# lyndonchan/wsss-analysis

Measured on AMD Instinct MI355X. Metric: images/sec CAM+CRF pseudo-labels, VOC2012 321x321, higher is better.
Workload: dtype f16x3; 1 GPU; resnet50 CAM + dense-CRF (M=21, 10 mean-field iters), 321x321, batch 32 images (=64 samples) per GPU, image-sharded; batch_images=32, num_classes=20, parallelism=image-sharded x1, no collective, steps_per_rank=239

## Files before the change

### include/wsscam.h

```cpp
#ifndef WSSCAM_H
#define WSSCAM_H

#include <stddef.h>
#include <stdint.h>

#ifdef __cplusplus
extern "C" {
#endif

#define WSC_VERSION 100

typedef enum wsc_status {
    WSC_OK = 0,
    WSC_ERR_INVALID = -1,
    WSC_ERR_NO_DEVICE = -2,
    WSC_ERR_HIP = -3,
    WSC_ERR_MISSING_KEY = -4,
    WSC_ERR_SHAPE = -5,
    WSC_ERR_NOMEM = -6,
    WSC_ERR_KEY_RANGE = -7,
    WSC_ERR_CAPACITY = -8,
    WSC_ERR_RANGE = -9
} wsc_status;

typedef enum wsc_arch {
    WSC_ARCH_RESNET50_CAM = 0,
    WSC_ARCH_VGG16_CAM = 1,
    WSC_ARCH_M7_CAM = 2,
    WSC_ARCH_RESNET50_IRN = 3,
    WSC_ARCH_VGG16_IRN = 4,
    WSC_ARCH_M7_IRN = 5,
    WSC_ARCH_DEEPLAB_LFOV = 6,
    WSC_ARCH_DEEPLAB_ASPP = 7
} wsc_arch;

typedef enum wsc_precision {
    WSC_PREC_BF16 = 0,
    WSC_PREC_BF16X3 = 1,
    WSC_PREC_F16 = 2,
    WSC_PREC_F16X3 = 3,
    WSC_PREC_F32 = 4
} wsc_precision;

typedef struct wsc_ctx wsc_ctx;
typedef struct wsc_net wsc_net;
typedef enum {
    WSC_OPT_CRF_GAUSS_ON_CHIP = 0,
    WSC_OPT_CRF_FUSED_BLUR = 1,
    WSC_OPT_CRF_BLUR_ON_CHIP = 2,
    WSC_OPT_CRF_RANK_BALLOT = 3,
    WSC_OPT_CRF_EMBED_FULL = 4,
    WSC_OPT_RW_TILED = 5,
    WSC_OPT_STEM_POOL_FUSED = 6,
    WSC_OPT_CONV_WINDOW = 7,
    WSC_OPT_CAM_HEAD_STREAM = 8,
    WSC_OPT_CRF_MSG_IN_UPDATE = 9,
    WSC_OPT_COUNT = 10
} wsc_option;

typedef struct wsc_crf wsc_crf;
typedef struct wsc_crf_v wsc_crf_v;

typedef struct wsc_tensor_desc {
    const char *name;
    const float *data;
    int32_t ndim;
    int64_t shape[4];
} wsc_tensor_desc;


int wsc_version(void);
const char *wsc_last_error(void);

int wsc_ctx_create(int device, void *stream, wsc_ctx **out);
void wsc_ctx_destroy(wsc_ctx *ctx);
int wsc_ctx_set_option(wsc_ctx *ctx, int option, int value);
int wsc_sync(wsc_ctx *ctx);
int wsc_ctx_range_status(wsc_ctx *ctx, int *flag_out, int clear);
int wsc_ctx_wait(wsc_ctx *ctx, wsc_ctx *other);
int wsc_ctx_mark(wsc_ctx *ctx, int slot);
int wsc_ctx_wait_mark(wsc_ctx *ctx, int slot);
int wsc_ctx_wait_for_mark(wsc_ctx *ctx, wsc_ctx *other, int slot);
int wsc_device_info(wsc_ctx *ctx, char *arch_name, size_t arch_name_len, int *num_cus);

int wsc_malloc(wsc_ctx *ctx, size_t bytes, void **dptr_out);
int wsc_free(wsc_ctx *ctx, void *dptr);
int wsc_memcpy_h2d(wsc_ctx *ctx, void *dst_dev, const void *src_host, size_t bytes);
int wsc_memcpy_d2h(wsc_ctx *ctx, void *dst_host, const void *src_dev, size_t bytes);
int wsc_memset(wsc_ctx *ctx, void *dst_dev, int value, size_t bytes);
int wsc_host_alloc(wsc_ctx *ctx, size_t bytes, void **host_out);
int wsc_host_free(wsc_ctx *ctx, void *host);
int wsc_host_write_segments(const char *path, int n, const void *const *ptrs, const size_t *sizes);
int wsc_memcpy_h2d_async(wsc_ctx *ctx, void *dst_dev, const void *src_pinned_host, size_t bytes);
int wsc_memcpy_d2h_async(wsc_ctx *ctx, void *dst_pinned_host, const void *src_dev, size_t bytes);

int wsc_timer_begin(wsc_ctx *ctx);
int wsc_timer_end(wsc_ctx *ctx, float *ms_out);

int wsc_profile_begin(wsc_ctx *ctx);
int wsc_profile_end(wsc_ctx *ctx, int max_classes, int32_t *calls_out, float *total_ms_out, double *work_out,
                    int *n_classes_out);
const char *wsc_profile_class_name(int cls);


int wsc_net_create(wsc_ctx *ctx, int arch, const wsc_tensor_desc *weights, int n_weights,
                   int num_classes, int precision, wsc_net **out);
void wsc_net_destroy(wsc_net *net);
int wsc_net_cam_size(const wsc_net *net, int S, int *h_out);
int wsc_net_feat_channels(const wsc_net *net, int *f_out);

int wsc_net_forward_cam(wsc_ctx *ctx, const wsc_net *net, const float *x_dev, int B, int S,
                        float *cam_dev, float *score_dev);
int wsc_net_cam_size_hw(const wsc_net *net, int H, int W, int *h_out, int *w_out);
int wsc_net_forward_cam_hw(wsc_ctx *ctx, const wsc_net *net, const float *x_dev, int B, int H, int W, float *cam_dev,
                           float *score_dev);

int wsc_net_forward_features(wsc_ctx *ctx, const wsc_net *net, const float *x_dev ,
                             int N, int S, float *feat_dev);

int wsc_net_forward_edge(wsc_ctx *ctx, const wsc_net *net, const float *x_dev, int B, int S, int feat_h, int feat_w,
                         float *edge_dev, float *dp_dev);
int wsc_net_edge_size(const wsc_net *net, int S, int *edge_hw, int *dp_hw);
int wsc_net_forward_edge_raw(wsc_ctx *ctx, const wsc_net *net, const float *x_dev, int N, int S, float *edge_dev, float *dp_dev);

int wsc_rw_propagate(wsc_ctx *ctx, const float *x_dev, const float *edge_dev, int K, int h, int w,
                     const int32_t *dirs_host, const int32_t *path_start_host, const int32_t *path_yx_host, int D,
                     float beta, int n_steps, float *rw_dev);
int wsc_rw_propagate_batch(wsc_ctx *ctx, int n_img, const int32_t *K_host, const int32_t *h_host,
                           const int32_t *w_host, const float *x_dev, const float *edge_dev,
                           const int32_t *dirs_host, const int32_t *path_start_host, const int32_t *path_yx_host,
                           int D, float beta, int n_steps, float *rw_dev);

int wsc_net_forward_gradcam(wsc_ctx *ctx, const wsc_net *net, const float *x_dev, int N, int S, int relu,
                            float *cams_dev, float *score_dev);

#define WSC_CONV_GENERIC 0x100
int wsc_conv2d_nchw(wsc_ctx *ctx, const float *x_dev, int N, int Cin, int H, int W, const float *w_host,
                    int Cout, int kh, int kw, int stride, int pad, const float *scale_host,
                    const float *shift_host, const float *residual_dev, int relu, int precision,
                    float *y_dev);
// ... 246 lines not shown
```

### wsss-analysis_amd/csrc/common.h

```cpp
#pragma once
#include <hip/hip_runtime.h>
#include <assert.h>
#include <stdint.h>
#include <map>
#include <string>
#include <unordered_map>
#include <vector>

#include "../../include/wsscam.h"

typedef uint16_t bf16_t;

typedef __bf16 bf16x8_t __attribute__((ext_vector_type(8)));
typedef _Float16 f16x8_t __attribute__((ext_vector_type(8)));
typedef float f32x16_t __attribute__((ext_vector_type(16)));
typedef float f32x4_t __attribute__((ext_vector_type(4)));

__host__ __device__ inline bf16_t f32_to_bf16(float f) {
    union { float f; uint32_t u; } v;
    v.f = f;
    uint32_t u = v.u;
    if ((u & 0x7fffffffu) > 0x7f800000u) return (bf16_t)((u >> 16) | 0x40);
    u += 0x7fffu + ((u >> 16) & 1u);
    return (bf16_t)(u >> 16);
// ... 33 lines not shown
__host__ __device__ inline float f16_to_f32(uint16_t h) {
#if defined(__HIP_DEVICE_COMPILE__)
    return (float)__builtin_bit_cast(_Float16, h);
#else
    union { float f; uint32_t u; } o, magic;
    magic.u = 113u << 23;
    const uint32_t shifted_exp = 0x7c00u << 13;
    o.u = ((uint32_t)h & 0x7fffu) << 13;
    const uint32_t exp = shifted_exp & o.u;
    o.u += (127u - 15u) << 23;
    if (exp == shifted_exp) o.u += (128u - 16u) << 23;
    else if (exp == 0) { o.u += 1u << 23; o.f -= magic.f; }
    o.u |= ((uint32_t)h & 0x8000u) << 16;
    return o.f;
#endif
}
__host__ __device__ inline uint16_t f32_to_h16(float f, int fmt) { return fmt ? f32_to_f16(f) : f32_to_bf16(f); }
__host__ __device__ inline float h16_to_f32(uint16_t h, int fmt) { return fmt ? f16_to_f32(h) : bf16_to_f32(h); }

void wsc_set_error(const char *fmt, ...);
#define WSC_HIP(expr)                                                                          \
    do {                                                                                       \
        hipError_t _e = (expr);                                                                \
        if (_e != hipSuccess) {                                                                \
            wsc_set_error("%s:%d: %s failed: %s", __FILE__, __LINE__, #expr,                   \
                          hipGetErrorString(_e));                                              \
            return WSC_ERR_HIP;                                                                \
        }                                                                                      \
    } while (0)
#define WSC_CHECK(cond, code, ...)                                                             \
    do {                                                                                       \
        if (!(cond)) {                                                                         \
            wsc_set_error(__VA_ARGS__);                                                        \
            return (code);                                                                     \
        }                                                                                      \
    } while (0)
#define WSC_TRY(expr)                                                                          \
    do {                                                                                       \
        int _s = (expr);                                                                       \
        if (_s != WSC_OK) return _s;                                                           \
    } while (0)

enum WscKernelClass {
    WSC_K_CONV256 = 0,
    WSC_K_CONV128,
    WSC_K_CONV64,
    WSC_K_CONV_SMALLCIN,
    WSC_K_POOL_MISC,
    WSC_K_CAM_TAIL,
    WSC_K_CRF_BUILD,
    WSC_K_GAUSS_MSG,
    WSC_K_BLUR,
    WSC_K_SLICE_UPDATE,
    WSC_K_CRF_MISC,
    WSC_K_WGRAD,
    WSC_K_GRAD_MISC,
    WSC_K_COUNT
};
struct WscProfRecord {
    int cls;
    double work;
    hipEvent_t e0, e1;
};

struct WscGaussCache;
void wsc_gauss_cache_destroy(WscGaussCache *cache);
struct wsc_ctx {
    int device = 0;
    hipStream_t stream = nullptr;
    bool own_stream = false;
    int num_cus = 0;
    std::string arch;
    void *ws = nullptr;
    size_t ws_bytes = 0;
    static constexpr int PIN_SLOTS = 8;
    struct PinSlot {
        void *p = nullptr;
        size_t bytes = 0;
        hipEvent_t ev = nullptr;
        bool busy = false;
    };
    PinSlot pin_ring[PIN_SLOTS];
    int pin_next = 0;
    int opt[WSC_OPT_COUNT] = {1, 1, 1, 0, 0, -1, 1, 1, 1, 1};
    void *zero_page = nullptr;
    unsigned *range_host = nullptr, *range_dev = nullptr;
    hipEvent_t ev0 = nullptr, ev1 = nullptr;
    hipEvent_t join_ev = nullptr;
    hipEvent_t marks[8] = {};
    bool mark_set[8] = {};
    hipStream_t aux_stream = nullptr;
    hipEvent_t fork_ev = nullptr, aux_done_ev = nullptr;
    bool profiling = false;
    std::vector<WscProfRecord> prof;
    std::vector<hipEvent_t> prof_pool;
    std::multimap<size_t, void *> free_blocks;
    std::unordered_map<void *, size_t> live_blocks;
    WscGaussCache *gauss_cache = nullptr;
};
int wsc_ctx_workspace(wsc_ctx *ctx, size_t bytes, void **out);
int wsc_ctx_range_check(wsc_ctx *ctx);
__device__ __forceinline__ unsigned half2_at_ceiling(unsigned hw) { return (hw & 0x7fff7fffu) + 0x04010401u; }
struct WscKernelTimer {
    wsc_ctx *ctx;
    int idx = -1;
    WscKernelTimer(wsc_ctx *c, int cls, double work);
    ~WscKernelTimer();
};
int wsc_ctx_cached_alloc(wsc_ctx *ctx, size_t bytes, void **out);
void wsc_ctx_cached_free(wsc_ctx *ctx, void *p);
struct WscCachedGuard {
    wsc_ctx *ctx;
    void *p;
    WscCachedGuard(wsc_ctx *c, void *q) : ctx(c), p(q) {}
    WscCachedGuard(const WscCachedGuard &) = delete;
    WscCachedGuard &operator=(const WscCachedGuard &) = delete;
    void free_now() {
        if (p) wsc_ctx_cached_free(ctx, p);
        p = nullptr;
    }
    ~WscCachedGuard() { free_now(); }
};
int wsc_ctx_upload_small(wsc_ctx *ctx, void *dst_dev, const void *src_host, size_t bytes);
class WscStagedTable {
  public:
    explicit WscStagedTable(wsc_ctx *c) : ctx(c) {}
    WscStagedTable(const WscStagedTable &) = delete;
    WscStagedTable &operator=(const WscStagedTable &) = delete;
    ~WscStagedTable() { release(); }
    size_t add(const void *src, size_t bytes);
    template <class T> size_t add(const std::vector<T> &v) { return add(v.data(), v.size() * sizeof(T)); }
    int upload();
    template <class T> T *at(size_t off) const { return reinterpret_cast<T *>(dev + off); }
    int read_back(size_t off, void *dst, size_t bytes);
    void release() { wsc_ctx_cached_free(ctx, dev); dev = nullptr; }
  private:
    wsc_ctx *ctx;
    std::vector<char> host;
    char *dev = nullptr;
};
template <int NV> __device__ __forceinline__ void block_sum(double (&v)[NV], double *scratch) {
#pragma unroll
    for (int k = 0; k < NV; ++k)
        for (int off = 32; off > 0; off >>= 1) v[k] += __shfl_xor(v[k], off, 64);
    const int wave = threadIdx.x >> 6, n_waves = blockDim.x >> 6;
    __syncthreads();
    if ((threadIdx.x & 63) == 0)
        for (int k = 0; k < NV; ++k) scratch[wave * NV + k] = v[k];
    __syncthreads();
#pragma unroll
    for (int k = 0; k < NV; ++k) {
        double s = 0.0;
        for (int w = 0; w < n_waves; ++w) s += scratch[w * NV + k];
        v[k] = s;
    }
}

int wsc_set_max_dynamic_lds(wsc_ctx *ctx, const void *fn, int bytes);

constexpr int CONV_FMT_F32 = 2;
inline int conv_fmt(wsc_precision prec) {
    if (prec == WSC_PREC_F32) return CONV_FMT_F32;
    return (prec == WSC_PREC_F16 || prec == WSC_PREC_F16X3) ? 1 : 0;
}
inline size_t conv_elem_bytes(wsc_precision prec) { return prec == WSC_PREC_F32 ? sizeof(float) : sizeof(bf16_t); }
inline int conv_split(wsc_precision prec) { return prec == WSC_PREC_BF16X3 ? 1 : (prec == WSC_PREC_F16X3 ? 2 : 0); }

// ... 262 lines not shown
```

### wsss-analysis_amd/csrc/crf.hip

```cpp
#include "common.h"

#include <atomic>
#include <cmath>
#include <cstring>
#include <memory>

namespace {

constexpr unsigned long long EMPTY_KEY = 0xFFFFFFFFFFFFFFFFull;
typedef float f32x2_t __attribute__((ext_vector_type(2)));

struct LatticeDev {
    int d = 0;
    int rep = 1;
    int rows = 0;
    int32_t *offset = nullptr;
    float *bary = nullptr;
    float *norm = nullptr;
    int2 *nbr = nullptr;
    int32_t *tslot_start = nullptr;
    int2 *slot_desc = nullptr;
    float *tent_w = nullptr;
    uint8_t *tent_p = nullptr;
    int32_t *row_slot_start = nullptr;
    int n_tiles = 0, n_slots = 0;
    bool sorted_dest = false;
    long long n_pix = 0;
    int M_cur = 0;
    float alpha = 0.f;
    int32_t *tile_rows = nullptr;
    int2 *tile_pstart = nullptr;
    int32_t *tile_list = nullptr;
    int n_tiles_occ = 0;
    int4 *gt_cnt = nullptr;
    int2 *gt_rows = nullptr;
    uint4 *gt_nbr = nullptr;
    uint4 *gt_pix = nullptr;
    int gt_stride = 0;
    std::vector<int32_t> v_per_image;
    int32_t *img_row = nullptr;
    int max_img_rows = 0;
    uint32_t *part_row = nullptr;
    bool bl_ok = false;
    int2 *bl_blk = nullptr;
    int bl_cap = 0;
    mutable std::vector<int2> bl_blk_host;
    mutable int bl_M = -1, bl_nblk = 0;
    mutable size_t bl_lds = 0;
};

constexpr int TILE_W = 16, TILE_H = 16, TILE_PIX = TILE_W * TILE_H;
static_assert(TILE_PIX <= 256, "an entry's pixel index is stored in one byte");
constexpr int SLOT_ENT = 32;
constexpr int SORT_MAX = 2048;
static_assert(TILE_PIX * 6 <= SORT_MAX && SORT_MAX <= 65535, "tile too large for the in-LDS grouping");

struct TileGeom {
    int H, W, ntx, nty, tpi;
};
__host__ __device__ inline TileGeom make_geom(int H, int W) {
    TileGeom g;
    g.H = H; g.W = W;
    g.ntx = (W + TILE_W - 1) / TILE_W;
    g.nty = (H + TILE_H - 1) / TILE_H;
    g.tpi = g.ntx * g.nty;
    return g;
}
struct TileBox {
    int x0, y0, cw, ch;
    int ebase;
};
__host__ __device__ inline TileBox tile_box(const TileGeom &g, int j) {
    const unsigned ty = (unsigned)j / (unsigned)g.ntx, tx = (unsigned)j - ty * (unsigned)g.ntx;
    TileBox b;
    b.x0 = (int)(tx * (unsigned)g.W / (unsigned)g.ntx);
    b.y0 = (int)(ty * (unsigned)g.H / (unsigned)g.nty);
    b.cw = (int)((tx + 1) * (unsigned)g.W / (unsigned)g.ntx) - b.x0;
    b.ch = (int)((ty + 1) * (unsigned)g.H / (unsigned)g.nty) - b.y0;
    b.ebase = b.y0 * g.W + b.x0 * b.ch;
    return b;
}
static_assert(TILE_W <= 26 && TILE_PIX <= 4096, "tile_div_magic range");
__host__ __device__ inline unsigned tile_div_magic(int cw) { return (65536u + (unsigned)cw - 1u) / (unsigned)cw; }

struct CtxBlocks {
    wsc_ctx *ctx;
    std::vector<void *> ptrs;
    explicit CtxBlocks(wsc_ctx *c) : ctx(c) {}
    CtxBlocks(CtxBlocks &&o) noexcept : ctx(o.ctx), ptrs(std::move(o.ptrs)) { o.ptrs.clear(); }
    ~CtxBlocks() { release(); }
    template <class T>
    int alloc(size_t bytes, T **out) {
        void *p = nullptr;
        WSC_TRY(wsc_ctx_cached_alloc(ctx, bytes, &p));
        ptrs.push_back(p);
        *out = static_cast<T *>(p);
        return WSC_OK;
    }
    void take(CtxBlocks &&o) {
        ptrs.insert(ptrs.end(), o.ptrs.begin(), o.ptrs.end());
        o.ptrs.clear();
    }
    void release() {
        for (void *p : ptrs) wsc_ctx_cached_free(ctx, p);
        ptrs.clear();
    }
};

struct GaussEntry {
    int H, W;
    float sxy;
    LatticeDev L;
    CtxBlocks blocks;
    int users = 0;
    unsigned long long last_use = 0;
    bool fuse_pending = true;
};
constexpr int GAUSS_CACHE_MAX = 64;
std::atomic<unsigned long long> g_gauss_use_clock{0};

}

struct wsc_crf {
    wsc_ctx *ctx = nullptr;
    int B = 0, H = 0, W = 0, N = 0;
    LatticeDev lat[2];
    uint4 *pix_rec = nullptr;
    uint32_t *pix_rec_b = nullptr;
    CtxBlocks blocks;
    GaussEntry *gauss = nullptr;
// ... 899 lines not shown
                        while (hi - lo > 1) {
                            const int mid = (lo + hi) >> 1;
                            if (rss_l[mid] <= pp) lo = mid;
                            else hi = mid;
                        }
                        single = rss_l[lo + 1] - rss_l[lo] == 1;
                    }
                    if (single) {
                        val[(unsigned)(r0 + lo) * (unsigned)LP + l] = v[u];
                    } else {
#pragma unroll
                        for (int k = 0; k < 4; ++k)
                            atomicAdd(&acc[lo * 32 + 4 * l + k], (unsigned long long)(long long)__float2int_rn(v[u][k] * PFIX_SCALE));
                    }
                }
            }
        }
    }
    __syncthreads();
    if (tr < gpb) {
        for (int row = tr; row < nr; row += gpb) {
            const int n = rss_l[row + 1] - rss_l[row];
            if (n == 1) continue;
            f32x4_t o = {0.f, 0.f, 0.f, 0.f};
            if (n > 1) {
#pragma unroll
                for (int k = 0; k < 4; ++k) o[k] = (float)(long long)acc[row * 32 + 4 * l + k] * PFIX_INV;
            }
            val[(unsigned)(r0 + row) * (unsigned)LP + l] = o;
        }
    }
}


__global__ __launch_bounds__(256) void blur1_kernel(const float *__restrict__ in, const int2 *__restrict__ nbr,
                                                    int rows, float *__restrict__ out) {
    for (int row = blockIdx.x * blockDim.x + threadIdx.x; row < rows; row += gridDim.x * blockDim.x) {
        const int2 nb = nbr[row];
        out[row] = row == 0 ? 0.f : in[row] + 0.5f * (in[nb.x] + in[nb.y]);
    }
}

__global__ __launch_bounds__(256) void blur4_kernel(const f32x4_t *__restrict__ in, const int2 *__restrict__ nbr,
                                                    int LP, int rows_local, int rep, f32x4_t *__restrict__ out) {
    const int rpb = 256 / LP;
    const int tr = threadIdx.x / LP;
    const int l = threadIdx.x - tr * LP;
    if (tr >= rpb) return;
    constexpr int U = 4;
    long long rbeg, rend;
    int rk;
    xcd_range_rep(rows_local, rep, rk, rbeg, rend);
    in += (size_t)rk * rows_local * LP;
    out += (size_t)rk * rows_local * LP;
    for (long long row0 = rbeg + tr; row0 < rend; row0 += U * rpb) {
        int2 nb[U];
        f32x4_t c[U], a[U], b[U];
#pragma unroll
        for (int u = 0; u < U; ++u) {
            const long long row = row0 + u * rpb;
            nb[u] = row < rend ? nbr[row] : make_int2(0, 0);
        }
#pragma unroll
        for (int u = 0; u < U; ++u) {
            const long long row = row0 + u * rpb;
            c[u] = in[(unsigned)(row < rend ? row : 0) * (unsigned)LP + l];
            a[u] = in[(unsigned)nb[u].x * (unsigned)LP + l];
            b[u] = in[(unsigned)nb[u].y * (unsigned)LP + l];
        }
#pragma unroll
        for (int u = 0; u < U; ++u) {
            const long long row = row0 + u * rpb;
            if (row < rend) {
                f32x4_t o;
#pragma unroll
                for (int k = 0; k < 4; ++k) o[k] = row == 0 ? 0.f : c[u][k] + 0.5f * (a[u][k] + b[u][k]);
                out[(unsigned)row * (unsigned)LP + l] = o;
            }
        }
    }
}

constexpr int BL_THREADS = 1024;
constexpr int BL_NVAR = 5;
constexpr int BL_VAR[BL_NVAR][2] = {{4, 4}, {4, 10}, {3, 13}, {2, 20}, {1, 26}};
inline int blur_lds_variant(int rows) {
    for (int v = 0; v < BL_NVAR; ++v)
        if (rows <= BL_VAR[v][1] * BL_THREADS && (size_t)(rows + 1) * BL_VAR[v][0] * 4 <= 160 * 1024 && rows < 65535) return v;
    return -1;
}
struct BlurLdsArgs {
    const int2 *nbr;
    const int32_t *img_row;
    const int2 *blk;
    float *val;
    int Mp, M, rows, npass;
};
template <int GW> struct FloatRun { float v[GW]; };
typedef float f32x3u_t __attribute__((ext_vector_type(3), aligned(4)));
template <int GW>
__device__ __forceinline__ FloatRun<GW> load_run(const float *q) {
    FloatRun<GW> r;
    if constexpr (GW == 4) {
        const f32x4_t x = *reinterpret_cast<const f32x4_t *>(q);
        r.v[0] = x[0]; r.v[1] = x[1]; r.v[2] = x[2]; r.v[3] = x[3];
    } else if constexpr (GW == 3) {
        const f32x3u_t x = *reinterpret_cast<const f32x3u_t *>(q);
        r.v[0] = x[0]; r.v[1] = x[1]; r.v[2] = x[2];
    } else if constexpr (GW == 2) {
        const f32x2_t x = *reinterpret_cast<const f32x2_t *>(q);
        r.v[0] = x[0]; r.v[1] = x[1];
    } else {
        r.v[0] = q[0];
    }
    return r;
}
template <int GW>
__device__ __forceinline__ void store_run(float *q, const FloatRun<GW> &r) {
    if constexpr (GW == 4) *reinterpret_cast<f32x4_t *>(q) = f32x4_t{r.v[0], r.v[1], r.v[2], r.v[3]};
    else if constexpr (GW == 3) {
        f32x3u_t x;
        x[0] = r.v[0]; x[1] = r.v[1]; x[2] = r.v[2];
        *reinterpret_cast<f32x3u_t *>(q) = x;
    } else if constexpr (GW == 2) *reinterpret_cast<f32x2_t *>(q) = f32x2_t{r.v[0], r.v[1]};
    else q[0] = r.v[0];
}
template <int GW, int RPT>
__device__ __forceinline__ void blur_lds_body(const BlurLdsArgs &p, float *pl, int img, int grp) {
    const int r0 = p.img_row[img], nr = p.img_row[img + 1] - r0;
    const int stride = nr + 1;
    const int c0 = grp * GW;
    const int tid = (int)threadIdx.x;
    float *vb = p.val + (size_t)r0 * p.Mp + c0;
    unsigned nb[RPT];
    auto load_idx = [&](int pass) {
        const int2 *q = p.nbr + (size_t)pass * p.rows + r0;
        constexpr int CH = RPT < 10 ? RPT : 10;
#pragma unroll
        for (int i0 = 0; i0 < RPT; i0 += CH) {
            int2 raw[CH];
#pragma unroll
            for (int i = 0; i < CH; ++i) {
                const int r = tid + (i0 + i) * BL_THREADS;
                raw[i] = (i0 + i < RPT && r < nr) ? q[r] : make_int2(0, 0);
            }
#pragma unroll
            for (int i = 0; i < CH; ++i)
                if (i0 + i < RPT)
                    nb[i0 + i] = (unsigned)(raw[i].x ? raw[i].x - r0 : nr) | ((unsigned)(raw[i].y ? raw[i].y - r0 : nr) << 16);
        }
    };
    load_idx(0);
#pragma unroll
    for (int i = 0; i < RPT; ++i) {
        const int r = tid + i * BL_THREADS;
        if (r < nr) {
            FloatRun<GW> run;
            if (GW == 3 && c0 + GW > p.Mp) {
#pragma unroll
                for (int g = 0; g < GW; ++g) run.v[g] = c0 + g < p.Mp ? vb[(size_t)r * p.Mp + g] : 0.f;
            } else {
                run = load_run<GW>(vb + (size_t)r * p.Mp);
            }
#pragma unroll
            for (int g = 0; g < GW; ++g) pl[g * stride + r] = c0 + g < p.M ? run.v[g] : 0.f;
        }
    }
    if (tid < GW) pl[tid * stride + nr] = 0.f;
    __syncthreads();
    float o[RPT][GW];
    for (int pass = 0; pass < p.npass; ++pass) {
#pragma unroll
        for (int i = 0; i < RPT; ++i) {
            const int r = tid + i * BL_THREADS;
            const int rc = r < nr ? r : nr;
            const int l1 = (int)(nb[i] & 0xffffu), l2 = (int)(nb[i] >> 16);
#pragma unroll
            for (int g = 0; g < GW; ++g) o[i][g] = pl[g * stride + rc] + 0.5f * (pl[g * stride + l1] + pl[g * stride + l2]);
        }
        if (pass + 1 < p.npass) load_idx(pass + 1);
        else break;
        __syncthreads();
#pragma unroll
        for (int i = 0; i < RPT; ++i) {
            const int r = tid + i * BL_THREADS;
            if (r < nr) {
#pragma unroll
                for (int g = 0; g < GW; ++g) pl[g * stride + r] = o[i][g];
            }
        }
        __syncthreads();
    }
#pragma unroll
    for (int i = 0; i < RPT; ++i) {
        const int r = tid + i * BL_THREADS;
        if (r < nr) {
            if (c0 + GW <= p.M) {
                FloatRun<GW> run;
#pragma unroll
                for (int g = 0; g < GW; ++g) run.v[g] = o[i][g];
                store_run<GW>(vb + (size_t)r * p.Mp, run);
            } else {
#pragma unroll
                for (int g = 0; g < GW; ++g)
                    if (c0 + g < p.M) vb[(size_t)r * p.Mp + g] = o[i][g];
            }
        }
    }
}
__global__ __launch_bounds__(BL_THREADS) void blur_lds_kernel(BlurLdsArgs p) {
    extern __shared__ float pl[];
    const int2 w = p.blk[blockIdx.x];
    if (w.x < 0) return;
    const int img = w.x & 0xffffff;
    switch (w.x >> 24) {
    case 0: blur_lds_body<BL_VAR[0][0], BL_VAR[0][1]>(p, pl, img, w.y); break;
    case 1: blur_lds_body<BL_VAR[1][0], BL_VAR[1][1]>(p, pl, img, w.y); break;
    case 2: blur_lds_body<BL_VAR[2][0], BL_VAR[2][1]>(p, pl, img, w.y); break;
    case 3: blur_lds_body<BL_VAR[3][0], BL_VAR[3][1]>(p, pl, img, w.y); break;
    default: blur_lds_body<BL_VAR[4][0], BL_VAR[4][1]>(p, pl, img, w.y); break;
    }
}

constexpr int GTI = 12, GTJ = 12, GBI = GTI + 4, GBJ = GTJ + 4;
constexpr int GLH = 6;

__global__ void gauss_ij_kernel(const unsigned long long *__restrict__ rowkey, int rows, int2 *__restrict__ ij,
                                int *__restrict__ bbox ) {
    for (int row = 1 + blockIdx.x * blockDim.x + threadIdx.x; row < rows; row += gridDim.x * blockDim.x) {
        int key[2];
        unpack_key<2>(rowkey[row], key);
        const int a = 2 * key[0] + key[1], b = key[0] + 2 * key[1];
        if (a % 3 != 0 || b % 3 != 0) atomicOr(&bbox[4], 1);
        const int i = a / 3, j = b / 3;
        ij[row] = make_int2(i, j);
        atomicMin(&bbox[0], i);
        atomicMin(&bbox[1], j);
        atomicMax(&bbox[2], i);
        atomicMax(&bbox[3], j);
    }
}

__global__ void gauss_tile_fill_kernel(const int2 *__restrict__ ij, int rows, int imin, int jmin, int nti, int ntj,
                                       int32_t *__restrict__ tile_rows, int32_t *__restrict__ occ) {
    for (int row = 1 + blockIdx.x * blockDim.x + threadIdx.x; row < rows; row += gridDim.x * blockDim.x) {
        const int i = ij[row].x - imin, j = ij[row].y - jmin;
        occ[(i / GTI) * ntj + j / GTJ] = 1;
        for (int ti = (i - GTI - 1 >= 0 ? (i - GTI - 1) / GTI : 0); ti <= (i + 2) / GTI && ti < nti; ++ti) {
            const int li = i - ti * GTI + 2;
            if (li < 0 || li >= GBI) continue;
            for (int tj = (j - GTJ - 1 >= 0 ? (j - GTJ - 1) / GTJ : 0); tj <= (j + 2) / GTJ && tj < ntj; ++tj) {
                const int lj = j - tj * GTJ + 2;
                if (lj < 0 || lj >= GBJ) continue;
                tile_rows[((long long)ti * ntj + tj) * (GBI * GBJ) + li * GBJ + lj] = row;
            }
        }
    }
}

__global__ void gauss_tile_pstart_kernel(const int32_t *__restrict__ tile_rows, const int32_t *__restrict__ row_slot_start,
                                         long long total, int2 *__restrict__ tile_pstart) {
    for (long long i = (long long)blockIdx.x * blockDim.x + threadIdx.x; i < total; i += (long long)gridDim.x * blockDim.x) {
        const int row = tile_rows[i];
        tile_pstart[i] = row ? make_int2(row_slot_start[row], row_slot_start[row + 1] - row_slot_start[row]) : make_int2(0, 0);
    }
}

__global__ __launch_bounds__(GBI * GBJ) void blur3_tile_kernel(const f32x4_t *__restrict__ in, const int32_t *__restrict__ tile_rows,
                                                         const int32_t *__restrict__ tile_list, int n_occ, int LP,
                                                         int rows_local, int rep, f32x4_t *__restrict__ out,
                                                         const f32x4_t *__restrict__ part, const int2 *__restrict__ tile_pstart,
                                                         int n_slots) {
    constexpr int P = GBI * GBJ;
    constexpr int PS = P + 1;
    __shared__ f32x4_t b0[GLH * PS];
    const int nb = gridDim.x, bid = blockIdx.x;
    const int xcd = bid & 7, qq = nb >> 3, rr = nb & 7;
    const int lb = (xcd < rr ? xcd * (qq + 1) : rr * (qq + 1) + (xcd - rr) * qq) + (bid >> 3);
    const int k = lb / n_occ, t = lb - k * n_occ;
    if (in) in += (size_t)k * rows_local * LP;
    if (part) part += (size_t)k * n_slots * LP;
    out += (size_t)k * rows_local * LP;
    const int p = threadIdx.x;
    const int li = p / GBJ, lj = p - li * GBJ;
    const long long tbase = (long long)tile_list[t] * P;
    const int row = tile_rows[tbase + p];
    const f32x4_t zero = {0.f, 0.f, 0.f, 0.f};
    if (t == 0 && p < LP) out[p] = zero;
    const bool r0 = row && li >= 1 && li < GBI - 1;
    const bool r1 = r0 && lj >= 1 && lj < GBJ - 1;
    const bool r2 = row && li >= 2 && li < GBI - 2 && lj >= 2 && lj < GBJ - 2;
    int prow[GLH], psb[GLH], pse[GLH];
#pragma unroll
    for (int i = 0; i < GLH; ++i) {
        const int pp = (i * P + p) / GLH;
        const int pli = pp / GBJ, plj = pp - pli * GBJ;
        const int r = tile_rows[tbase + pp];
        psb[i] = 0; pse[i] = 0;
        if (part && r) {
            const int2 ps = tile_pstart[tbase + pp];
            psb[i] = ps.x;
            pse[i] = ps.x + ps.y;
        }
        prow[i] = (r && pli >= 2 && pli < GBI - 2 && plj >= 2 && plj < GBJ - 2) ? r : (r ? -r : 0);
// ... 931 lines not shown
        }
        *reinterpret_cast<f32x4_t *>(dst + m0) = v;
    }
}

__global__ __launch_bounds__(TP) void finish_kernel(const float *__restrict__ q, int M, int Mp, int N,
                                                    float *__restrict__ q_out, int32_t *__restrict__ argmax) {
    extern __shared__ float tile[];
    const int b = blockIdx.y;
    const int n0 = blockIdx.x * TP;
    const int np = min(TP, N - n0);
    const long long ibase = ((long long)b * N + n0) * Mp;
    for (int i = threadIdx.x; i < np * Mp; i += TP) {
        const int n = i / Mp, m = i - n * Mp;
        if (m < M) tile[m * (TP + 1) + n] = q[ibase + i];
    }
    __syncthreads();
    if ((int)threadIdx.x < np) {
        if (q_out)
            for (int m = 0; m < M; ++m)
                q_out[((long long)b * M + m) * N + n0 + threadIdx.x] = tile[m * (TP + 1) + threadIdx.x];
        if (argmax) {
            int best = 0;
            float bv = tile[threadIdx.x];
            for (int m = 1; m < M; ++m) {
                const float v = tile[m * (TP + 1) + threadIdx.x];
                if (v > bv) {
                    bv = v;
                    best = m;
                }
            }
            argmax[(long long)b * N + n0 + threadIdx.x] = best;
        }
    }
}

__global__ void fill_tables_kernel(unsigned long long *__restrict__ table, unsigned *__restrict__ first, long long n) {
    for (long long i = (long long)blockIdx.x * blockDim.x + threadIdx.x; i < n; i += (long long)gridDim.x * blockDim.x) {
        table[i] = EMPTY_KEY;
        first[i] = 0x7fffffffu;
    }
}

inline int grid1d(long long total, int per_block = 256, int cap = 256 * 32) {
    long long g = (total + per_block - 1) / per_block;
    if (g > cap) g = cap;
    if (g < 1) g = 1;
    return (int)g;
}

inline int grid_rep(long long total, int per_block, int rep) {
    const int g = grid1d(total, per_block, 256 * 64);
    return g <= rep ? rep : g / rep * rep;
}

void splat_ones(wsc_ctx *ctx, const LatticeDev &L, const TileGeom &tg, float *val, float *part) {
    hipLaunchKernelGGL(slot_ones_kernel, dim3((unsigned)L.n_tiles), dim3(256), 0, ctx->stream, L.tslot_start, L.slot_desc,
                       L.tent_w, L.d + 1, tg, part);
    hipLaunchKernelGGL(combine1_kernel, dim3(grid1d(L.rows)), dim3(256), 0, ctx->stream, part, L.row_slot_start, L.rows, val);
}

void combine4(wsc_ctx *ctx, hipStream_t st, const LatticeDev &L, const float *part, int LP, float *val) {
    WscKernelTimer timer(ctx, WSC_K_BLUR, ((double)L.n_slots + L.rows) * L.rep * L.M_cur * 4);
    if (L.sorted_dest)
        hipLaunchKernelGGL(combine4_kernel, dim3(grid_rep((long long)L.rows * L.rep, 256 / LP, L.rep)), dim3(256), 0,
                           st, (const f32x4_t *)part, L.row_slot_start, LP, L.rows, L.n_slots, L.rep, (f32x4_t *)val);
    else
        hipLaunchKernelGGL(combine4_balanced_kernel, dim3((unsigned)((L.rows + CB_ROWS - 1) / CB_ROWS)), dim3(256), 0, st,
                           (const f32x4_t *)part, L.row_slot_start, (const uint32_t *)L.part_row, LP, L.rows, (f32x4_t *)val);
}

float *blur_all1(wsc_ctx *ctx, const LatticeDev &L, float *a, float *b) {
    for (int j = 0; j <= L.d; ++j) {
        hipLaunchKernelGGL(blur1_kernel, dim3(grid1d(L.rows)), dim3(256), 0, ctx->stream, a,
                           L.nbr + (long long)j * L.rows, L.rows, b);
        float *t = a; a = b; b = t;
    }
    return a;
}

int blur_lds_prepare(wsc_ctx *ctx, const LatticeDev &L, int M) {
    if (L.rep != 1 || !L.img_row || !L.bl_ok) return WSC_OK;
    const int B = (int)L.v_per_image.size();
    if (L.bl_M != M) {
        std::vector<std::vector<int2>> q(8);
        size_t lds = 0;
        for (int b = 0; b < B; ++b) {
            const int v = blur_lds_variant(L.v_per_image[b]), gw = BL_VAR[v][0];
            lds = std::max(lds, (size_t)(L.v_per_image[b] + 1) * gw * 4);
            for (int g = 0; g * gw < M; ++g) q[b & 7].push_back(make_int2(b | (v << 24), g));
        }
        size_t len = 0;
        for (int x = 0; x < 8; ++x) len = std::max(len, q[x].size());
        std::vector<int2> &h = L.bl_blk_host;
        h.assign(len * 8, make_int2(-1, 0));
        for (int x = 0; x < 8; ++x)
            for (size_t i = 0; i < q[x].size(); ++i) h[i * 8 + x] = q[x][i];
        L.bl_M = -1;
        if ((int)h.size() > L.bl_cap) return WSC_OK;
        WSC_TRY(wsc_ctx_upload_small(ctx, L.bl_blk, h.data(), sizeof(int2) * h.size()));
        L.bl_nblk = (int)h.size();
        L.bl_lds = lds;
        L.bl_M = M;
    }
    return WSC_OK;
}
bool blur_lds(wsc_ctx *ctx, hipStream_t st, const LatticeDev &L, int LP, float *val) {
    const int M = L.M_cur;
    if (!ctx->opt[WSC_OPT_CRF_BLUR_ON_CHIP] || L.rep != 1 || !L.img_row || !L.bl_ok || L.bl_M != M) return false;
    if (L.bl_nblk == 0) return true;
    if (wsc_set_max_dynamic_lds(ctx, reinterpret_cast<const void *>(blur_lds_kernel), 160 * 1024) != WSC_OK) return false;
    BlurLdsArgs ba;
    ba.nbr = L.nbr; ba.img_row = L.img_row; ba.blk = L.bl_blk; ba.val = val; ba.Mp = 4 * LP; ba.M = M; ba.rows = L.rows;
    ba.npass = L.d + 1;
    WscKernelTimer timer(ctx, WSC_K_BLUR, 2.0 * (L.d + 1) * L.rows * M * 4);
    hipLaunchKernelGGL(blur_lds_kernel, dim3((unsigned)L.bl_nblk), dim3(BL_THREADS), L.bl_lds, st, ba);
    return true;
}

float *combine_blur_all4(wsc_ctx *ctx, hipStream_t st, const LatticeDev &L, int LP, const float *part, float *a, float *b) {
    const bool fused_off = !ctx->opt[WSC_OPT_CRF_FUSED_BLUR];
    if (L.d == 2 && L.tile_rows && L.tile_pstart && L.n_tiles_occ > 0 && !fused_off) {
        WscKernelTimer timer(ctx, WSC_K_BLUR, ((double)L.n_slots + L.rows) * L.rep * L.M_cur * 4);
        hipLaunchKernelGGL(blur3_tile_kernel, dim3((unsigned)(L.n_tiles_occ * L.rep)), dim3(GBI * GBJ), 0, st,
                           (const f32x4_t *)nullptr, L.tile_rows, L.tile_list, L.n_tiles_occ, LP, L.rows, L.rep, (f32x4_t *)b,
                           (const f32x4_t *)part, L.tile_pstart, L.n_slots);
        return b;
    }
    combine4(ctx, st, L, part, LP, a);
    if (blur_lds(ctx, st, L, LP, a)) return a;
    for (int j = 0; j <= L.d; ++j) {
        WscKernelTimer timer(ctx, WSC_K_BLUR, 2.0 * L.rows * L.rep * L.M_cur * 4);
        hipLaunchKernelGGL(blur4_kernel, dim3(grid_rep((long long)L.rows * L.rep, (256 / LP) * 4, L.rep)), dim3(256),
                           0, st, (const f32x4_t *)a, L.nbr + (long long)j * L.rows, LP, L.rows, L.rep,
                           (f32x4_t *)b);
        float *t = a; a = b; b = t;
    }
    return a;
}

constexpr int GT_MAX_LOCAL = 1022;
int gauss_fuse_tables(wsc_ctx *ctx, const TileGeom &tg, LatticeDev &L, CtxBlocks &own) {
    const int N = tg.H * tg.W, rows = L.rows, W = tg.W;
    std::vector<int32_t> off((size_t)N * 3), rss((size_t)rows + 1);
    std::vector<float> bary((size_t)N * 3), norm((size_t)N);
    std::vector<int2> nbr((size_t)3 * rows);
    WSC_HIP(hipMemcpyAsync(off.data(), L.offset, sizeof(int32_t) * off.size(), hipMemcpyDeviceToHost, ctx->stream));
    WSC_HIP(hipMemcpyAsync(bary.data(), L.bary, sizeof(float) * bary.size(), hipMemcpyDeviceToHost, ctx->stream));
    WSC_HIP(hipMemcpyAsync(norm.data(), L.norm, sizeof(float) * norm.size(), hipMemcpyDeviceToHost, ctx->stream));
    WSC_HIP(hipMemcpyAsync(rss.data(), L.row_slot_start, sizeof(int32_t) * rss.size(), hipMemcpyDeviceToHost, ctx->stream));
    WSC_HIP(hipMemcpyAsync(nbr.data(), L.nbr, sizeof(int2) * nbr.size(), hipMemcpyDeviceToHost, ctx->stream));
    WSC_HIP(hipStreamSynchronize(ctx->stream));
    std::vector<int> loc((size_t)rows, -1);
    std::vector<std::vector<int>> sets((size_t)tg.tpi);
    std::vector<int4> cnt((size_t)tg.tpi);
    int nvmax = 0;
    for (int j = 0; j < tg.tpi; ++j) {
        const TileBox tb = tile_box(tg, j);
        std::vector<int> &list = sets[j];
        auto add = [&](int R) {
            if (R > 0 && R < rows && loc[R] < 0) {
                loc[R] = (int)list.size();
                list.push_back(R);
            }
        };
        for (int ty = 0; ty < tb.ch; ++ty)
            for (int tx = 0; tx < tb.cw; ++tx) {
                const size_t n = (size_t)(tb.y0 + ty) * W + tb.x0 + tx;
                for (int r = 0; r < 3; ++r) add(off[n * 3 + r]);
            }
        int4 &c = cnt[j];
        c.x = (int)list.size();
        for (int axis = 2; axis >= 0; --axis) {
            const size_t cur = list.size();
            for (size_t i = 0; i < cur; ++i) {
                const int2 nb = nbr[(size_t)axis * rows + list[i]];
                add(nb.x);
                add(nb.y);
            }
            if (axis == 2) c.y = (int)list.size();
            if (axis == 1) c.z = (int)list.size();
        }
        c.w = (int)list.size();
        for (int R : list) loc[R] = -1;
        if ((int)list.size() > nvmax) nvmax = (int)list.size();
    }
    if (nvmax > GT_MAX_LOCAL || nvmax == 0) return WSC_OK;
    const int stride = nvmax + 1, zr = stride - 1;
    std::vector<int2> trows((size_t)tg.tpi * stride, make_int2(0, 0));
    std::vector<uint4> tnbr((size_t)tg.tpi * stride, make_uint4((unsigned)zr | ((unsigned)zr << 16), (unsigned)zr | ((unsigned)zr << 16),
                                                                (unsigned)zr | ((unsigned)zr << 16), 0u));
    std::vector<uint4> pix((size_t)N);
    for (int j = 0; j < tg.tpi; ++j) {
        const TileBox tb = tile_box(tg, j);
        const std::vector<int> &list = sets[j];
        const int nv = (int)list.size();
        for (int v = 0; v < nv; ++v) loc[list[v]] = v;
        auto lid = [&](int R) { return (R > 0 && R < rows && loc[R] >= 0) ? loc[R] : zr; };
        for (int v = 0; v < nv; ++v) {
// ... 711 lines not shown
```

### wsss-analysis_amd/wsscam/_lib.py

```python
import ctypes
import os
import re
import threading

import numpy as np

_HERE = os.path.dirname(os.path.abspath(__file__))
LIB_PATH = os.path.join(_HERE, "libwsscam.so")
HEADER_PATH = os.path.normpath(os.path.join(_HERE, "..", "..", "include", "wsscam.h"))

WSC_OK = 0
WSC_ERR_INVALID = -1
WSC_ERR_NO_DEVICE = -2
WSC_ERR_HIP = -3
WSC_ERR_MISSING_KEY = -4
WSC_ERR_SHAPE = -5
WSC_ERR_NOMEM = -6
WSC_ERR_KEY_RANGE = -7
WSC_ERR_CAPACITY = -8
WSC_ERR_RANGE = -9

ARCH_RESNET50_CAM = 0
ARCH_VGG16_CAM = 1
ARCH_M7_CAM = 2
ARCH_RESNET50_IRN = 3
ARCH_VGG16_IRN = 4
ARCH_M7_IRN = 5
ARCH_DEEPLAB_LFOV = 6
ARCH_DEEPLAB_ASPP = 7

PREC_BF16 = 0
PREC_BF16X3 = 1
PREC_F16 = 2
PREC_F16X3 = 3
PREC_F32 = 4
OPT_CRF_GAUSS_ON_CHIP, OPT_CRF_FUSED_BLUR, OPT_CRF_BLUR_ON_CHIP, OPT_CRF_RANK_BALLOT, OPT_CRF_EMBED_FULL, OPT_RW_TILED, \
    OPT_STEM_POOL_FUSED, OPT_CONV_WINDOW, OPT_CAM_HEAD_STREAM, OPT_CRF_MSG_IN_UPDATE = range(10)
OPT_DEFAULTS = {OPT_CRF_GAUSS_ON_CHIP: 1, OPT_CRF_FUSED_BLUR: 1, OPT_CRF_BLUR_ON_CHIP: 1, OPT_CRF_RANK_BALLOT: 0,
                OPT_CRF_EMBED_FULL: 0, OPT_RW_TILED: -1, OPT_STEM_POOL_FUSED: 1, OPT_CONV_WINDOW: 1, OPT_CAM_HEAD_STREAM: 1,
                OPT_CRF_MSG_IN_UPDATE: 1}
CONV_GENERIC = 0x100


class WscError(RuntimeError):
    def __init__(self, status, message):
        super().__init__("libwsscam error %d: %s" % (status, message))
        self.status = status


class TensorDesc(ctypes.Structure):
    _fields_ = [
        ("name", ctypes.c_char_p),
        ("data", ctypes.POINTER(ctypes.c_float)),
        ("ndim", ctypes.c_int32),
        ("shape", ctypes.c_int64 * 4),
    ]


class TraceOp(ctypes.Structure):
    _fields_ = [(n, ctypes.c_int32) for n in (
        "kind", "in_", "in2", "res", "Ho", "Wo", "C", "coff", "pitch", "kh", "kw", "stride", "pad", "dil", "relu", "affine2", "stride2",
        "pool_rule", "pool_k", "pool_stride", "pool_pad", "pool_avg", "fused_next")] + [("label", ctypes.c_char * 100)]


class TapeEntry(ctypes.Structure):
    _fields_ = [("name", ctypes.c_char * 32), ("Ho", ctypes.c_int32), ("Wo", ctypes.c_int32), ("C", ctypes.c_int32),
                ("offset", ctypes.c_int64)]


class GradEntry(ctypes.Structure):
    _fields_ = [("name", ctypes.c_char * 32), ("kh", ctypes.c_int32), ("kw", ctypes.c_int32), ("Cin", ctypes.c_int32),
                ("Cout", ctypes.c_int32), ("w_off", ctypes.c_int64), ("b_off", ctypes.c_int64)]


TRACE_CONV, TRACE_POOL, TRACE_GATHER, TRACE_HEAD = range(4)
TRACE_INPUT, TRACE_NONE = -1, -2

_lib = None

_vp = ctypes.c_void_p
_i = ctypes.c_int
_f = ctypes.c_float
_sz = ctypes.c_size_t
_d = ctypes.c_double

_SIGNATURES = {
    "wsc_version": (_i, []),
    "wsc_last_error": (ctypes.c_char_p, []),
    "wsc_ctx_create": (_i, [_i, _vp, ctypes.POINTER(_vp)]),
    "wsc_ctx_destroy": (None, [_vp]),
    "wsc_sync": (_i, [_vp]),
    "wsc_ctx_range_status": (_i, [_vp, ctypes.POINTER(_i), _i]),
    "wsc_ctx_wait": (_i, [_vp, _vp]),
    "wsc_ctx_mark": (_i, [_vp, _i]),
    "wsc_ctx_wait_mark": (_i, [_vp, _i]),
    "wsc_ctx_wait_for_mark": (_i, [_vp, _vp, _i]),
    "wsc_device_info": (_i, [_vp, ctypes.c_char_p, _sz, ctypes.POINTER(_i)]),
    "wsc_malloc": (_i, [_vp, _sz, ctypes.POINTER(_vp)]),
    "wsc_free": (_i, [_vp, _vp]),
    "wsc_memcpy_h2d": (_i, [_vp, _vp, _vp, _sz]),
    "wsc_memcpy_d2h": (_i, [_vp, _vp, _vp, _sz]),
    "wsc_memset": (_i, [_vp, _vp, _i, _sz]),
    "wsc_ctx_set_option": (_i, [_vp, _i, _i]),
    "wsc_host_alloc": (_i, [_vp, _sz, ctypes.POINTER(_vp)]),
    "wsc_host_free": (_i, [_vp, _vp]),
    "wsc_host_write_segments": (_i, [ctypes.c_char_p, _i, ctypes.POINTER(_vp), ctypes.POINTER(_sz)]),
    "wsc_memcpy_h2d_async": (_i, [_vp, _vp, _vp, _sz]),
    "wsc_memcpy_d2h_async": (_i, [_vp, _vp, _vp, _sz]),
    "wsc_profile_begin": (_i, [_vp]),
    "wsc_profile_end": (_i, [_vp, _i, _vp, _vp, _vp, ctypes.POINTER(_i)]),
    "wsc_profile_class_name": (ctypes.c_char_p, [_i]),
    "wsc_timer_begin": (_i, [_vp]),
    "wsc_timer_end": (_i, [_vp, ctypes.POINTER(_f)]),
    "wsc_net_create": (_i, [_vp, _i, ctypes.POINTER(TensorDesc), _i, _i, _i, ctypes.POINTER(_vp)]),
    "wsc_net_destroy": (None, [_vp]),
    "wsc_net_cam_size": (_i, [_vp, _i, ctypes.POINTER(_i)]),
    "wsc_net_feat_channels": (_i, [_vp, ctypes.POINTER(_i)]),
    "wsc_net_forward_cam": (_i, [_vp, _vp, _vp, _i, _i, _vp, _vp]),
    "wsc_net_forward_gradcam": (_i, [_vp, _vp, _vp, _i, _i, _i, _vp, _vp]),
    "wsc_net_forward_features": (_i, [_vp, _vp, _vp, _i, _i, _vp]),
    "wsc_net_cam_size_hw": (_i, [_vp, _i, _i, ctypes.POINTER(_i), ctypes.POINTER(_i)]),
    "wsc_net_forward_cam_hw": (_i, [_vp, _vp, _vp, _i, _i, _i, _vp, _vp]),
    "wsc_net_forward_edge": (_i, [_vp, _vp, _vp, _i, _i, _i, _i, _vp, _vp]),
# ... 1067 lines not shown
```

Baseline: 2664 images/s.

## Store LDS blur lattice values row-interleaved and specialize per rows-per-thread

Adds a row-interleaved LDS layout for the on-chip lattice blur, so each row's group of channels is read and written as one vector LDS access instead of strided planar accesses. It also adds a variant for every rows-per-thread count from 1 to 26, which lets the bounds checks on the first RPT-2 iterations be dropped at compile time. The planar path stays behind a new option, and the row layout is on by default. The extra template instantiations grow code size and may raise register pressure, and the row layout can introduce LDS bank conflicts on random neighbour gathers.

```diff
diff --git a/include/wsscam.h b/include/wsscam.h
--- a/include/wsscam.h
+++ b/include/wsscam.h
@@ -55,7 +55,8 @@
     WSC_OPT_CONV_WINDOW = 7,
     WSC_OPT_CAM_HEAD_STREAM = 8,
     WSC_OPT_CRF_MSG_IN_UPDATE = 9,
-    WSC_OPT_COUNT = 10
+    WSC_OPT_CRF_BLUR_ROWS = 10,
+    WSC_OPT_COUNT = 11
 } wsc_option;
 
 typedef struct wsc_crf wsc_crf;
diff --git a/wsss-analysis_amd/csrc/common.h b/wsss-analysis_amd/csrc/common.h
--- a/wsss-analysis_amd/csrc/common.h
+++ b/wsss-analysis_amd/csrc/common.h
@@ -139,7 +139,7 @@
     };
     PinSlot pin_ring[PIN_SLOTS];
     int pin_next = 0;
-    int opt[WSC_OPT_COUNT] = {1, 1, 1, 0, 0, -1, 1, 1, 1, 1};
+    int opt[WSC_OPT_COUNT] = {1, 1, 1, 0, 0, -1, 1, 1, 1, 1, 1};
     void *zero_page = nullptr;
     unsigned *range_host = nullptr, *range_dev = nullptr;
     hipEvent_t ev0 = nullptr, ev1 = nullptr;
diff --git a/wsss-analysis_amd/csrc/crf.hip b/wsss-analysis_amd/csrc/crf.hip
--- a/wsss-analysis_amd/csrc/crf.hip
+++ b/wsss-analysis_amd/csrc/crf.hip
@@ -46,6 +46,7 @@
     int bl_cap = 0;
     mutable std::vector<int2> bl_blk_host;
     mutable int bl_M = -1, bl_nblk = 0;
+    mutable bool bl_row_layout = true;
     mutable size_t bl_lds = 0;
 };
 
@@ -1111,11 +1112,23 @@
 }
 
 constexpr int BL_THREADS = 1024;
-constexpr int BL_NVAR = 5;
-constexpr int BL_VAR[BL_NVAR][2] = {{4, 4}, {4, 10}, {3, 13}, {2, 20}, {1, 26}};
-inline int blur_lds_variant(int rows) {
+constexpr int BL_NVAR = 26;
+constexpr int BL_VAR[BL_NVAR][2] = {{4, 1},  {4, 2},  {4, 3},  {4, 4},  {4, 5},  {4, 6},  {4, 7},  {4, 8},  {4, 9},
+                                    {4, 10}, {3, 11}, {3, 12}, {3, 13}, {2, 14}, {2, 15}, {2, 16}, {2, 17}, {2, 18},
+                                    {2, 19}, {2, 20}, {1, 21}, {1, 22}, {1, 23}, {1, 24}, {1, 25}, {1, 26}};
+constexpr bool bl_var_consecutive() {
     for (int v = 0; v < BL_NVAR; ++v)
-        if (rows <= BL_VAR[v][1] * BL_THREADS && (size_t)(rows + 1) * BL_VAR[v][0] * 4 <= 160 * 1024 && rows < 65535) return v;
+        if (BL_VAR[v][1] != v + 1) return false;
+    return true;
+}
+static_assert(bl_var_consecutive(), "BL_VAR: every RPT from 1 up, in order");
+constexpr int BL_NPLANAR = 5;
+constexpr int BL_PLANAR[BL_NPLANAR][2] = {{4, 4}, {4, 10}, {3, 13}, {2, 20}, {1, 26}};
+inline int blur_lds_variant(int rows, bool row_layout = true) {
+    const int n = row_layout ? BL_NVAR : BL_NPLANAR;
+    const int(*var)[2] = row_layout ? BL_VAR : BL_PLANAR;
+    for (int v = 0; v < n; ++v)
+        if (rows <= var[v][1] * BL_THREADS && (size_t)(rows + 1) * var[v][0] * 4 <= 160 * 1024 && rows < 65535) return v;
     return -1;
 }
 struct BlurLdsArgs {
@@ -1154,13 +1167,40 @@
     } else if constexpr (GW == 2) *reinterpret_cast<f32x2_t *>(q) = f32x2_t{r.v[0], r.v[1]};
     else q[0] = r.v[0];
 }
-template <int GW, int RPT>
+template <int GW, int RPT, bool ROWL>
 __device__ __forceinline__ void blur_lds_body(const BlurLdsArgs &p, float *pl, int img, int grp) {
     const int r0 = p.img_row[img], nr = p.img_row[img + 1] - r0;
     const int stride = nr + 1;
     const int c0 = grp * GW;
     const int tid = (int)threadIdx.x;
     float *vb = p.val + (size_t)r0 * p.Mp + c0;
+    if (ROWL && nr <= (RPT - 2) * BL_THREADS) return;
+    auto has = [&](int i, int r) { return (ROWL && i < RPT - 2) || r < nr; };
+    constexpr int WA = GW == 3 ? 2 : GW, WB = GW - WA;
+    float *pb = pl + WA * stride;
+    auto lds_get = [&](int r, float *v) {
+        if constexpr (ROWL) {
+            const FloatRun<WA> a = load_run<WA>(pl + r * WA);
+#pragma unroll
+            for (int g = 0; g < WA; ++g) v[g] = a.v[g];
+            if constexpr (WB == 1) v[WA] = pb[r];
+        } else {
+#pragma unroll
+            for (int g = 0; g < GW; ++g) v[g] = pl[g * stride + r];
+        }
+    };
+    auto lds_put = [&](int r, const float *v) {
+        if constexpr (ROWL) {
+            FloatRun<WA> a;
+#pragma unroll
+            for (int g = 0; g < WA; ++g) a.v[g] = v[g];
+            store_run<WA>(pl + r * WA, a);
+            if constexpr (WB == 1) pb[r] = v[WA];
+        } else {
+#pragma unroll
+            for (int g = 0; g < GW; ++g) pl[g * stride + r] = v[g];
+        }
+    };
     unsigned nb[RPT];
     auto load_idx = [&](int pass) {
         const int2 *q = p.nbr + (size_t)pass * p.rows + r0;
@@ -1171,7 +1211,7 @@
 #pragma unroll
             for (int i = 0; i < CH; ++i) {
                 const int r = tid + (i0 + i) * BL_THREADS;
-                raw[i] = (i0 + i < RPT && r < nr) ? q[r] : make_int2(0, 0);
+                raw[i] = (i0 + i < RPT && has(i0 + i, r)) ? q[r] : make_int2(0, 0);
             }
 #pragma unroll
             for (int i = 0; i < CH; ++i)
@@ -1183,7 +1223,7 @@
 #pragma unroll
     for (int i = 0; i < RPT; ++i) {
         const int r = tid + i * BL_THREADS;
-        if (r < nr) {
+        if (has(i, r)) {
             FloatRun<GW> run;
             if (GW == 3 && c0 + GW > p.Mp) {
 #pragma unroll
@@ -1192,20 +1232,28 @@
                 run = load_run<GW>(vb + (size_t)r * p.Mp);
             }
 #pragma unroll
-            for (int g = 0; g < GW; ++g) pl[g * stride + r] = c0 + g < p.M ? run.v[g] : 0.f;
-        }
-    }
-    if (tid < GW) pl[tid * stride + nr] = 0.f;
+            for (int g = 0; g < GW; ++g) run.v[g] = c0 + g < p.M ? run.v[g] : 0.f;
+            lds_put(r, run.v);
+        }
+    }
+    if (tid == 0) {
+        const float z[4] = {0.f, 0.f, 0.f, 0.f};
+        lds_put(nr, z);
+    }
     __syncthreads();
     float o[RPT][GW];
     for (int pass = 0; pass < p.npass; ++pass) {
 #pragma unroll
         for (int i = 0; i < RPT; ++i) {
             const int r = tid + i * BL_THREADS;
-            const int rc = r < nr ? r : nr;
+            const int rc = has(i, r) ? r : nr;
             const int l1 = (int)(nb[i] & 0xffffu), l2 = (int)(nb[i] >> 16);
-#pragma unroll
-            for (int g = 0; g < GW; ++g) o[i][g] = pl[g * stride + rc] + 0.5f * (pl[g * stride + l1] + pl[g * stride + l2]);
+            float c[GW], x1[GW], x2[GW];
+            lds_get(rc, c);
+            lds_get(l1, x1);
+            lds_get(l2, x2);
+#pragma unroll
+            for (int g = 0; g < GW; ++g) o[i][g] = c[g] + 0.5f * (x1[g] + x2[g]);
         }
         if (pass + 1 < p.npass) load_idx(pass + 1);
         else break;
@@ -1213,42 +1261,50 @@
 #pragma unroll
         for (int i = 0; i < RPT; ++i) {
             const int r = tid + i * BL_THREADS;
-            if (r < nr) {
-#pragma unroll
-                for (int g = 0; g < GW; ++g) pl[g * stride + r] = o[i][g];
-            }
+            if (has(i, r)) lds_put(r, o[i]);
         }
         __syncthreads();
     }
+    int mp = p.Mp;
+    asm volatile("" : "+s"(mp));
 #pragma unroll
     for (int i = 0; i < RPT; ++i) {
         const int r = tid + i * BL_THREADS;
-        if (r < nr) {
+        if (has(i, r)) {
             if (c0 + GW <= p.M) {
                 FloatRun<GW> run;
 #pragma unroll
                 for (int g = 0; g < GW; ++g) run.v[g] = o[i][g];
-                store_run<GW>(vb + (size_t)r * p.Mp, run);
+                store_run<GW>(vb + (size_t)r * mp, run);
             } else {
 #pragma unroll
                 for (int g = 0; g < GW; ++g)
-                    if (c0 + g < p.M) vb[(size_t)r * p.Mp + g] = o[i][g];
-            }
-        }
-    }
+                    if (c0 + g < p.M) vb[(size_t)r * mp + g] = o[i][g];
+            }
+        }
+    }
+}
+template <int V>
+__device__ __forceinline__ void blur_lds_rows(int v, const BlurLdsArgs &p, float *pl, int img, int grp) {
+    if (v == V || V + 1 == BL_NVAR) blur_lds_body<BL_VAR[V][0], BL_VAR[V][1], true>(p, pl, img, grp);
+    else if constexpr (V + 1 < BL_NVAR) blur_lds_rows<V + 1>(v, p, pl, img, grp);
+}
+template <int V>
+__device__ __forceinline__ void blur_lds_planar(int v, const BlurLdsArgs &p, float *pl, int img, int grp) {
+    if (v == V || V + 1 == BL_NPLANAR) blur_lds_body<BL_PLANAR[V][0], BL_PLANAR[V][1], false>(p, pl, img, grp);
+    else if constexpr (V + 1 < BL_NPLANAR) blur_lds_planar<V + 1>(v, p, pl, img, grp);
 }
 __global__ __launch_bounds__(BL_THREADS) void blur_lds_kernel(BlurLdsArgs p) {
-    extern __shared__ float pl[];
+    extern __shared__ __attribute__((aligned(16))) float pl[];
     const int2 w = p.blk[blockIdx.x];
     if (w.x < 0) return;
-    const int img = w.x & 0xffffff;
-    switch (w.x >> 24) {
-    case 0: blur_lds_body<BL_VAR[0][0], BL_VAR[0][1]>(p, pl, img, w.y); break;
-    case 1: blur_lds_body<BL_VAR[1][0], BL_VAR[1][1]>(p, pl, img, w.y); break;
-    case 2: blur_lds_body<BL_VAR[2][0], BL_VAR[2][1]>(p, pl, img, w.y); break;
-    case 3: blur_lds_body<BL_VAR[3][0], BL_VAR[3][1]>(p, pl, img, w.y); break;
-    default: blur_lds_body<BL_VAR[4][0], BL_VAR[4][1]>(p, pl, img, w.y); break;
-    }
+    blur_lds_rows<0>(w.x >> 24, p, pl, w.x & 0xffffff, w.y);
+}
+__global__ __launch_bounds__(BL_THREADS) void blur_lds_planar_kernel(BlurLdsArgs p) {
+    extern __shared__ __attribute__((aligned(16))) float pl[];
+    const int2 w = p.blk[blockIdx.x];
+    if (w.x < 0) return;
+    blur_lds_planar<0>(w.x >> 24, p, pl, w.x & 0xffffff, w.y);
 }
 
 constexpr int GTI = 12, GTJ = 12, GBI = GTI + 4, GBJ = GTJ + 4;
@@ -2346,11 +2402,12 @@
 int blur_lds_prepare(wsc_ctx *ctx, const LatticeDev &L, int M) {
     if (L.rep != 1 || !L.img_row || !L.bl_ok) return WSC_OK;
     const int B = (int)L.v_per_image.size();
-    if (L.bl_M != M) {
+    const bool rowl = ctx->opt[WSC_OPT_CRF_BLUR_ROWS] != 0;
+    if (L.bl_M != M || L.bl_row_layout != rowl) {
         std::vector<std::vector<int2>> q(8);
         size_t lds = 0;
         for (int b = 0; b < B; ++b) {
-            const int v = blur_lds_variant(L.v_per_image[b]), gw = BL_VAR[v][0];
+            const int v = blur_lds_variant(L.v_per_image[b], rowl), gw = rowl ? BL_VAR[v][0] : BL_PLANAR[v][0];
             lds = std::max(lds, (size_t)(L.v_per_image[b] + 1) * gw * 4);
             for (int g = 0; g * gw < M; ++g) q[b & 7].push_back(make_int2(b | (v << 24), g));
         }
@@ -2365,6 +2422,7 @@
         WSC_TRY(wsc_ctx_upload_small(ctx, L.bl_blk, h.data(), sizeof(int2) * h.size()));
         L.bl_nblk = (int)h.size();
         L.bl_lds = lds;
+        L.bl_row_layout = rowl;
         L.bl_M = M;
     }
     return WSC_OK;
@@ -2373,12 +2431,13 @@
     const int M = L.M_cur;
     if (!ctx->opt[WSC_OPT_CRF_BLUR_ON_CHIP] || L.rep != 1 || !L.img_row || !L.bl_ok || L.bl_M != M) return false;
     if (L.bl_nblk == 0) return true;
-    if (wsc_set_max_dynamic_lds(ctx, reinterpret_cast<const void *>(blur_lds_kernel), 160 * 1024) != WSC_OK) return false;
+    void (*const kern)(BlurLdsArgs) = L.bl_row_layout ? blur_lds_kernel : blur_lds_planar_kernel;
+    if (wsc_set_max_dynamic_lds(ctx, reinterpret_cast<const void *>(kern), 160 * 1024) != WSC_OK) return false;
     BlurLdsArgs ba;
     ba.nbr = L.nbr; ba.img_row = L.img_row; ba.blk = L.bl_blk; ba.val = val; ba.Mp = 4 * LP; ba.M = M; ba.rows = L.rows;
     ba.npass = L.d + 1;
     WscKernelTimer timer(ctx, WSC_K_BLUR, 2.0 * (L.d + 1) * L.rows * M * 4);
-    hipLaunchKernelGGL(blur_lds_kernel, dim3((unsigned)L.bl_nblk), dim3(BL_THREADS), L.bl_lds, st, ba);
+    hipLaunchKernelGGL(kern, dim3((unsigned)L.bl_nblk), dim3(BL_THREADS), L.bl_lds, st, ba);
     return true;
 }
 
diff --git a/wsss-analysis_amd/wsscam/_lib.py b/wsss-analysis_amd/wsscam/_lib.py
--- a/wsss-analysis_amd/wsscam/_lib.py
+++ b/wsss-analysis_amd/wsscam/_lib.py
@@ -35,10 +35,10 @@
 PREC_F16X3 = 3
 PREC_F32 = 4
 OPT_CRF_GAUSS_ON_CHIP, OPT_CRF_FUSED_BLUR, OPT_CRF_BLUR_ON_CHIP, OPT_CRF_RANK_BALLOT, OPT_CRF_EMBED_FULL, OPT_RW_TILED, \
-    OPT_STEM_POOL_FUSED, OPT_CONV_WINDOW, OPT_CAM_HEAD_STREAM, OPT_CRF_MSG_IN_UPDATE = range(10)
+    OPT_STEM_POOL_FUSED, OPT_CONV_WINDOW, OPT_CAM_HEAD_STREAM, OPT_CRF_MSG_IN_UPDATE, OPT_CRF_BLUR_ROWS = range(11)
 OPT_DEFAULTS = {OPT_CRF_GAUSS_ON_CHIP: 1, OPT_CRF_FUSED_BLUR: 1, OPT_CRF_BLUR_ON_CHIP: 1, OPT_CRF_RANK_BALLOT: 0,
                 OPT_CRF_EMBED_FULL: 0, OPT_RW_TILED: -1, OPT_STEM_POOL_FUSED: 1, OPT_CONV_WINDOW: 1, OPT_CAM_HEAD_STREAM: 1,
-                OPT_CRF_MSG_IN_UPDATE: 1}
+                OPT_CRF_MSG_IN_UPDATE: 1, OPT_CRF_BLUR_ROWS: 1}
 CONV_GENERIC = 0x100
 
 
```

Result: no change. 2669 images/s, median of 3 (+0.2%).
